# q8888620002/Group-Attribution-for-Diffusion-Models

Measured on AMD Instinct MI355X. Metric: shapley_coalitions_per_hour, higher is better.
Workload: dtype f32; 1 GPU; CIFAR-20 DDPM sFT coalition (BASELINE configs[1]): gd_steps=1000 @B=128 + 10240 samples x 100 DDIM steps @B=32 (32 batches fused/launch), UNet2DModel widths [128, 256, 256, 256] 35.75M params fp32; step = 1/1000 coalition = 1 train step + 1 sampler step @B=1024, enqueued on 3 HIP streams (the train step belongs to a later coalition: independent work); coalitions_in_flight=3

## Files before the change

group-attribution-for-diffusion-models_amd/csrc/norm.hip:

```cpp
#include "gad_common.h"
#include "gad_reduce.h"
#include "gemm_dev.h"

namespace {

constexpr int NT = 256;
constexpr int MAXC = 3072;

struct Geo {
  int B, HW, C, G, cpg, C4, tpr, rows_par, nch, ppc;
};

static Geo make_geo(const gad_groupnorm_args* a) {
  Geo g;
  g.B = a->B; g.HW = a->HW; g.C = a->C; g.G = a->G;
  g.cpg = a->C / a->G;
  g.C4 = a->C / 4;
  g.tpr = g.C4 < NT ? g.C4 : NT;
  g.rows_par = NT / g.tpr;
  int nch = 2048 / (a->B > 0 ? a->B : 1);
  int maxch = a->HW / (8 * g.rows_par > 32 ? 8 * g.rows_par : 32);
  if (nch > maxch) nch = maxch;
  if (nch < 1) nch = 1;
  g.ppc = (a->HW + nch - 1) / nch;
// ... 156 lines not shown
    f32x4 mu, rs;
#pragma unroll
    for (int e = 0; e < 4; ++e) {
      int grp = (c0 + e) / g.cpg;
      mu[e] = s_mean[grp];
      rs[e] = s_rstd[grp];
    }
    f32x4 scale = rs * ga, shift = be - mu * scale;
    const bool far = gn_far_mean(mu, rs);
    long base = ((long)b * g.HW) * g.C + c0;
    int ldx;
    const float* xb = gn_src(x, x2, C1, g.C, g.HW, b, c0, &ldx);
    int p = p0 + prow;
    const int R = g.rows_par;
    for (; p + 3 * R < p1; p += 4 * R) {
      f32x4 v[4];
#pragma unroll
      for (int u = 0; u < 4; ++u) v[u] = *reinterpret_cast<const f32x4*>(xb + (long)(p + u * R) * ldx);
#pragma unroll
      for (int u = 0; u < 4; ++u) {
        f32x4 z = far ? (v[u] - mu) * scale + be : v[u] * scale + shift;
        if (silu) {
#pragma unroll
          for (int e = 0; e < 4; ++e) z[e] = silu_f(z[e]);
        }
        *reinterpret_cast<f32x4*>(y + base + (long)(p + u * R) * g.C) = z;
      }
    }
    for (; p < p1; p += R) {
      f32x4 v = *reinterpret_cast<const f32x4*>(xb + (long)p * ldx);
      f32x4 z = far ? (v - mu) * scale + be : v * scale + shift;
      if (silu) {
#pragma unroll
        for (int e = 0; e < 4; ++e) z[e] = silu_f(z[e]);
      }
      *reinterpret_cast<f32x4*>(y + base + (long)p * g.C) = z;
    }
  }
}


struct SlabGeo {
  int HW, C, G, cpg, SC, qpr, PL, P2, nslab, gps, qpg;
  int xgrp;
};
__device__ __forceinline__ void slab_of_block(const SlabGeo& s, int& b, int& sl) {
  const int bid = blockIdx.x;
  if (s.xgrp) {
    const int x = bid & 7, r = bid >> 3;
    const int bp = r / s.nslab;
    sl = r - bp * s.nslab;
    b = bp * 8 + x;
  } else {
    b = bid / s.nslab;
    sl = bid - b * s.nslab;
  }
}

__device__ __forceinline__ void slab_reduce(float* red, float val, const SlabGeo& s, int pl, bool act) {
  red[threadIdx.x] = val;
  for (int st = s.P2 >> 1; st >= 1; st >>= 1) {
    __syncthreads();
    if (act && pl < st && pl + st < s.PL) red[threadIdx.x] += red[threadIdx.x + st * s.qpr];
  }
  __syncthreads();
}

template <int NTH>
__device__ __forceinline__ void slab_reduce4(f32x4* red, f32x4 val, const SlabGeo& s, int pl, bool act) {
  red[threadIdx.x] = val;
  for (int st = s.P2 >> 1; st >= 1; st >>= 1) {
    __syncthreads();
    if (act && pl < st && pl + st < s.PL) red[threadIdx.x] += red[threadIdx.x + st * s.qpr];
  }
  __syncthreads();
}

template <int NV, bool PERCH = false, int NTH = NT>
__global__ __launch_bounds__(NTH) void gn_slab_kernel(const float* __restrict__ x, const float* __restrict__ x2, int C1,
                                                     float* __restrict__ y,
                                                     const float* __restrict__ gamma, const float* __restrict__ beta,
                                                     float* __restrict__ mean_out, float* __restrict__ rstd_out,
                                                     SlabGeo s, float eps, int silu) {
  __shared__ float red[PERCH ? 4 : NTH];
  __shared__ f32x4 red4[PERCH ? NTH : 1];
  __shared__ float s_mean[64], s_rstd[64];
  int b, sl;
  slab_of_block(s, b, sl);
  const int tid = threadIdx.x;
  const int pl = tid / s.qpr, q = tid - pl * s.qpr;
  const bool act = pl < s.PL;
  const int c0 = sl * s.SC + q * 4;
  const long base = ((long)b * s.HW) * s.C + c0;
  const bool second = c0 >= C1;
  const int ldin = second ? s.C - C1 : C1;
  const float* xin = (second ? x2 + (c0 - C1) : x + c0) + ((long)b * s.HW) * ldin;
  f32x4 v[NV];
#pragma unroll
  for (int i = 0; i < NV; ++i) {
    int p = pl + i * s.PL;
    v[i] = (act && p < s.HW) ? *reinterpret_cast<const f32x4*>(xin + (long)p * ldin) : f32x4{0.f, 0.f, 0.f, 0.f};
  }
  f32x4 acc = {0.f, 0.f, 0.f, 0.f};
#pragma unroll
  for (int i = 0; i < NV; ++i) acc += v[i];
  const float inv_n = 1.f / (float)((long)s.HW * s.cpg);
  const float* chan = reinterpret_cast<const float*>(red4);
  int gi[4] = {0, 0, 0, 0};
  if (PERCH) {
#pragma unroll
    for (int e = 0; e < 4; ++e) gi[e] = act ? (q * 4 + e) / s.cpg : 0;
    slab_reduce4<NTH>(red4, acc, s, pl, act);
  } else {
    slab_reduce(red, (acc[0] + acc[1]) + (acc[2] + acc[3]), s, pl, act);
  }
  float S = 0.f;
  if (tid < s.gps) {
    if (PERCH) for (int j = 0; j < s.cpg; ++j) S += chan[tid * s.cpg + j];
    else for (int j = 0; j < s.qpg; ++j) S += red[tid * s.qpg + j];
    s_mean[tid] = S * inv_n;
  }
  __syncthreads();
  f32x4 mu;
  if (PERCH) mu = f32x4{s_mean[gi[0]], s_mean[gi[1]], s_mean[gi[2]], s_mean[gi[3]]};
  else { const float m1 = act ? s_mean[q / s.qpg] : 0.f; mu = f32x4{m1, m1, m1, m1}; }
  acc = f32x4{0.f, 0.f, 0.f, 0.f};
#pragma unroll
  for (int i = 0; i < NV; ++i) {
    int p = pl + i * s.PL;
    f32x4 d = v[i] - mu;
    if (act && p < s.HW) acc += d * d;
  }
  if (PERCH) {
    __syncthreads();
    slab_reduce4<NTH>(red4, acc, s, pl, act);
  } else {
    slab_reduce(red, (acc[0] + acc[1]) + (acc[2] + acc[3]), s, pl, act);
  }
  if (tid < s.gps) {
    float SS = 0.f;
    if (PERCH) for (int j = 0; j < s.cpg; ++j) SS += chan[tid * s.cpg + j];
    else for (int j = 0; j < s.qpg; ++j) SS += red[tid * s.qpg + j];
    float rs = rsqrtf(SS * inv_n + eps);
    if (!((s_mean[tid] * rs) * (s_mean[tid] * rs) <= GN_COND - 1.f)) {
      const float md = S / (float)((long)s.HW * s.cpg), d = s_mean[tid] - md;
      rs = rsqrtf(fmaxf(SS * inv_n - d * d, 0.f) + eps);
      s_mean[tid] = md;
    }
    s_rstd[tid] = rs;
    mean_out[b * s.G + sl * s.gps + tid] = s_mean[tid];
    rstd_out[b * s.G + sl * s.gps + tid] = rs;
  }
  __syncthreads();
  if (!act) return;
  f32x4 rs;
  if (PERCH) {
    rs = f32x4{s_rstd[gi[0]], s_rstd[gi[1]], s_rstd[gi[2]], s_rstd[gi[3]]};
    mu = f32x4{s_mean[gi[0]], s_mean[gi[1]], s_mean[gi[2]], s_mean[gi[3]]};
  } else {
    const float r1 = s_rstd[q / s.qpg], m1 = s_mean[q / s.qpg];
    rs = f32x4{r1, r1, r1, r1};
    mu = f32x4{m1, m1, m1, m1};
  }
  f32x4 ga = *reinterpret_cast<const f32x4*>(gamma + c0), be = *reinterpret_cast<const f32x4*>(beta + c0);
  f32x4 scale = ga * rs, shift = be - scale * mu;
  const bool far = gn_far_mean(mu, rs);
#pragma unroll
  for (int i = 0; i < NV; ++i) {
    int p = pl + i * s.PL;
    if (p < s.HW) {
      f32x4 z = far ? (v[i] - mu) * scale + be : v[i] * scale + shift;
      if (silu) {
#pragma unroll
        for (int e = 0; e < 4; ++e) z[e] = silu_f(z[e]);
      }
      *reinterpret_cast<f32x4*>(y + base + (long)p * s.C) = z;
    }
  }
}

static int make_slab(const gad_groupnorm_args* a, SlabGeo* out, const int nth = NT, const int maxnv = 32) {
  const int cpg = a->C / a->G;
  SlabGeo best{};
  int best_nv = 0;
  long best_score = -1;
  for (int k = 1; k * cpg <= a->C && k <= 64; ++k) {
    int SC = k * cpg;
    if (a->C % SC != 0 || SC % 4 != 0) continue;
    const bool lines = (SC * 4) % 128 == 0 || SC == a->C;
    if (!lines && (a->B % 8 != 0 || a->C / SC > 8 || (long)a->B * (a->C / SC) > 1024)) continue;
    int qpr = SC / 4;
    if (qpr > nth) break;
    int PL = nth / qpr;
    int nv = (a->HW + PL - 1) / PL;
    if (nv > maxnv) continue;
    long blocks = (long)a->B * (a->C / SC);
    long score = (blocks >= 1024 ? (1L << 40) : blocks << 16) + SC + (lines ? (1L << 41) : 0);
    if (score > best_score) {
      best_score = score;
      best_nv = nv;
      int P2 = 1;
      while (P2 < PL) P2 <<= 1;
      best = SlabGeo{a->HW, a->C, a->G, cpg, SC, qpr, PL, P2, a->C / SC, k, cpg / 4, lines ? 0 : 1};
    }
  }
  if (!best_nv) return 0;
  *out = best;
  return best_nv <= 4 ? 4 : best_nv <= 8 ? 8 : best_nv <= 16 ? 16 : 32;
}

struct GnWino {
  float* V;
  int W, TH, TW;
  long pos_stride;
};

template <int NV>
__global__ __launch_bounds__(512) void gn_wino4_kernel(const float* __restrict__ x, const float* __restrict__ x2, int C1,
                                                      const float* __restrict__ gamma, const float* __restrict__ beta,
                                                      float* __restrict__ mean_out, float* __restrict__ rstd_out,
                                                      SlabGeo s, float eps, int silu, GnWino w) {
  constexpr int NTH = 512;
  extern __shared__ __attribute__((aligned(16))) float gn_img[];
  __shared__ float red[NTH];
  __shared__ float s_mean[64], s_rstd[64];
  int b, sl;
  slab_of_block(s, b, sl);
  const int tid = threadIdx.x;
  const int pl = tid / s.qpr, q = tid - pl * s.qpr;
  const bool act = pl < s.PL;
  const int c0 = sl * s.SC + q * 4;
  const bool second = c0 >= C1;
  const int ldin = second ? s.C - C1 : C1;
  const float* xin = (second ? x2 + (c0 - C1) : x + c0) + ((long)b * s.HW) * ldin;
  f32x4 v[NV];
#pragma unroll
  for (int i = 0; i < NV; ++i) {
    int p = pl + i * s.PL;
    v[i] = (act && p < s.HW) ? *reinterpret_cast<const f32x4*>(xin + (long)p * ldin) : f32x4{0.f, 0.f, 0.f, 0.f};
  }
  f32x4 acc = {0.f, 0.f, 0.f, 0.f};
#pragma unroll
  for (int i = 0; i < NV; ++i) acc += v[i];
  const float inv_n = 1.f / (float)((long)s.HW * s.cpg);
  slab_reduce(red, (acc[0] + acc[1]) + (acc[2] + acc[3]), s, pl, act);
  float S = 0.f;
  if (tid < s.gps) {
    for (int j = 0; j < s.qpg; ++j) S += red[tid * s.qpg + j];
    s_mean[tid] = S * inv_n;
  }
  __syncthreads();
  const float m1 = act ? s_mean[q / s.qpg] : 0.f;
  const f32x4 mu = f32x4{m1, m1, m1, m1};
  acc = f32x4{0.f, 0.f, 0.f, 0.f};
#pragma unroll
  for (int i = 0; i < NV; ++i) {
    int p = pl + i * s.PL;
    f32x4 d = v[i] - mu;
    if (act && p < s.HW) acc += d * d;
  }
  slab_reduce(red, (acc[0] + acc[1]) + (acc[2] + acc[3]), s, pl, act);
  if (tid < s.gps) {
    float SS = 0.f;
    for (int j = 0; j < s.qpg; ++j) SS += red[tid * s.qpg + j];
    float rs = rsqrtf(SS * inv_n + eps);
    if (!((s_mean[tid] * rs) * (s_mean[tid] * rs) <= GN_COND - 1.f)) {
      const float md = S / (float)((long)s.HW * s.cpg), d = s_mean[tid] - md;
      rs = rsqrtf(fmaxf(SS * inv_n - d * d, 0.f) + eps);
      s_mean[tid] = md;
    }
    s_rstd[tid] = rs;
    mean_out[b * s.G + sl * s.gps + tid] = s_mean[tid];
    rstd_out[b * s.G + sl * s.gps + tid] = rs;
  }
  __syncthreads();
  f32x4* img4 = reinterpret_cast<f32x4*>(gn_img);
  if (act) {
    const float r1 = s_rstd[q / s.qpg], m2 = s_mean[q / s.qpg];
    const f32x4 rs = f32x4{r1, r1, r1, r1}, mu2 = f32x4{m2, m2, m2, m2};
    const f32x4 ga = *reinterpret_cast<const f32x4*>(gamma + c0), be = *reinterpret_cast<const f32x4*>(beta + c0);
    const f32x4 scale = ga * rs, shift = be - scale * mu2;
    const bool far = gn_far_mean(mu2, rs);
#pragma unroll
    for (int i = 0; i < NV; ++i) {
      int p = pl + i * s.PL;
      if (p < s.HW) {
        f32x4 z = far ? (v[i] - mu2) * scale + be : v[i] * scale + shift;
        if (silu) {
#pragma unroll
          for (int e = 0; e < 4; ++e) z[e] = silu_f(z[e]);
        }
        const int yy = p / w.W, xx = p - yy * w.W;
        img4[(yy * w.W + (xx ^ ((xx >> 2) & 1))) * s.qpr + q] = z;
      }
    }
  }
  __syncthreads();
  const int H = s.HW / w.W;
  const int items = w.TH * w.TW * s.qpr;
  for (int it = tid; it < items; it += NTH) {
    const int tile = it / s.qpr, qq = it - tile * s.qpr;
    const int ty = tile / w.TW, tx = tile - ty * w.TW;
    f32x4 t[6][6];
#pragma unroll
    for (int dx = 0; dx < 6; ++dx) {
      const int xx = 4 * tx - 1 + dx;
      const bool xok = xx >= 0 && xx < w.W;
      const int xs = xx ^ ((xx >> 2) & 1);
      f32x4 d[6], col[6];
#pragma unroll
      for (int dy = 0; dy < 6; ++dy) {
        const int yy = 4 * ty - 1 + dy;
        const bool ok = xok && yy >= 0 && yy < H;
        d[dy] = ok ? img4[(yy * w.W + xs) * s.qpr + qq] : f32x4{0.f, 0.f, 0.f, 0.f};
      }
      gadk::wino4_bt(d, col);
#pragma unroll
      for (int i = 0; i < 6; ++i) t[i][dx] = col[i];
    }
    float* out = w.V + ((long)b * (w.TH * w.TW) + tile) * s.C + sl * s.SC + qq * 4;
#pragma unroll
    for (int i = 0; i < 6; ++i) {
      f32x4 vv[6];
      gadk::wino4_bt(t[i], vv);
#pragma unroll
      for (int j = 0; j < 6; ++j) *reinterpret_cast<f32x4*>(out + (long)(6 * i + j) * w.pos_stride) = vv[j];
    }
  }
}

static int make_slab_wino(const gad_groupnorm_args* a, SlabGeo* out) {
  const int cpg = a->C / a->G, nth = 512;
  if (cpg % 4 != 0) return 0;
  int best_nv = 0;
  long best_score = -1;
  for (int k = 1; k * cpg <= a->C && k <= 64; ++k) {
    const int SC = k * cpg;
    if (a->C % SC != 0 || SC % 32 != 0) continue;
    if ((long)a->HW * SC * 4 > 128 * 1024) break;
    const int qpr = SC / 4;
    if (qpr > nth) break;
    const int PL = nth / qpr, nv = (a->HW + PL - 1) / PL;
    if (nv > 16) continue;
    const long blocks = (long)a->B * (a->C / SC);
    const long score = (blocks >= 512 ? (1L << 40) : blocks << 16) + SC;
    if (score > best_score) {
      best_score = score;
      best_nv = nv;
      int P2 = 1;
      while (P2 < PL) P2 <<= 1;
      *out = SlabGeo{a->HW, a->C, a->G, cpg, SC, qpr, PL, P2, a->C / SC, k, cpg / 4, 0};
    }
  }
  return !best_nv ? 0 : best_nv <= 4 ? 4 : best_nv <= 8 ? 8 : 16;
}

__device__ __forceinline__ float act_grad(float dy, float z, int silu) {
  if (!silu) return dy;
  float s = 1.f / (1.f + expf(-z));
  return dy * s * (1.f + z * (1.f - s));
}

template <int NV, int NTH>
__global__ __launch_bounds__(NTH) void gn_bwd_slab_kernel(const float* __restrict__ x, const float* __restrict__ dy,
                                                          float* __restrict__ dx, const float* __restrict__ gamma,
                                                          const float* __restrict__ beta, const float* __restrict__ mean,
                                                          const float* __restrict__ rstd, float* __restrict__ part,
                                                          SlabGeo s, int silu, const float* __restrict__ dx_add) {
  __shared__ f32x4 red_a[NTH], red_b[NTH];
  __shared__ float s_m1[64], s_m2[64];
  int b, sl;
  slab_of_block(s, b, sl);
  const int tid = threadIdx.x;
  const int pl = tid / s.qpr, q = tid - pl * s.qpr;
  const bool act = pl < s.PL;
  const int c0 = sl * s.SC + (act ? q : 0) * 4;
  const long base = ((long)b * s.HW) * s.C + c0;
  int gi[4];
  f32x4 mu, rs;
#pragma unroll
  for (int e = 0; e < 4; ++e) {
    gi[e] = ((act ? q : 0) * 4 + e) / s.cpg;
    mu[e] = mean[b * s.G + sl * s.gps + gi[e]];
    rs[e] = rstd[b * s.G + sl * s.gps + gi[e]];
  }
  const f32x4 ga = *reinterpret_cast<const f32x4*>(gamma + c0), be = *reinterpret_cast<const f32x4*>(beta + c0);
  f32x4 xh[NV], ge[NV];
  f32x4 sa = {0.f, 0.f, 0.f, 0.f}, sb = {0.f, 0.f, 0.f, 0.f};
#pragma unroll
  for (int i = 0; i < NV; ++i) {
    const int p = pl + i * s.PL;
    if (act && p < s.HW) {
      const f32x4 v = *reinterpret_cast<const f32x4*>(x + base + (long)p * s.C);
      const f32x4 d = *reinterpret_cast<const f32x4*>(dy + base + (long)p * s.C);
      xh[i] = (v - mu) * rs;
#pragma unroll
      for (int e = 0; e < 4; ++e) ge[i][e] = act_grad(d[e], xh[i][e] * ga[e] + be[e], silu);
      sa += ge[i];
      sb += ge[i] * xh[i];
    } else {
      xh[i] = f32x4{0.f, 0.f, 0.f, 0.f};
      ge[i] = f32x4{0.f, 0.f, 0.f, 0.f};
    }
  }
  slab_reduce4<NTH>(red_a, sa, s, pl, act);
  slab_reduce4<NTH>(red_b, sb, s, pl, act);
  if (tid < s.qpr) {
    const int c = sl * s.SC + tid * 4;
    float* o = part + ((long)b * s.C + c) * 2;
    const f32x4 A = red_a[tid], Bx = red_b[tid];
#pragma unroll
    for (int e = 0; e < 4; ++e) { o[2 * e] = A[e]; o[2 * e + 1] = Bx[e]; }
  }
  if (tid < s.gps) {
    const float inv_n = 1.f / (float)((long)s.HW * s.cpg);
    const float* ca = reinterpret_cast<const float*>(red_a);
    const float* cb = reinterpret_cast<const float*>(red_b);
    float s1 = 0.f, s2 = 0.f;
    for (int j = 0; j < s.cpg; ++j) {
      const int c = tid * s.cpg + j;
      const float gj = gamma[sl * s.SC + c];
      s1 += ca[c] * gj;
      s2 += cb[c] * gj;
    }
    s_m1[tid] = s1 * inv_n;
    s_m2[tid] = s2 * inv_n;
  }
  __syncthreads();
  if (!act) return;
  const f32x4 m1 = {s_m1[gi[0]], s_m1[gi[1]], s_m1[gi[2]], s_m1[gi[3]]}, m2 = {s_m2[gi[0]], s_m2[gi[1]], s_m2[gi[2]], s_m2[gi[3]]};
#pragma unroll
  for (int i = 0; i < NV; ++i) {
    const int p = pl + i * s.PL;
    if (p < s.HW) {
      f32x4 o;
#pragma unroll
      for (int e = 0; e < 4; ++e) o[e] = rs[e] * (ge[i][e] * ga[e] - m1[e] - xh[i][e] * m2[e]);
      if (dx_add) o += *reinterpret_cast<const f32x4*>(dx_add + base + (long)p * s.C);
      *reinterpret_cast<f32x4*>(dx + base + (long)p * s.C) = o;
    }
  }
}

__global__ __launch_bounds__(NT) void gn_bwd_stats_kernel(const float* __restrict__ x, const float* __restrict__ dy,
                                                          const float* __restrict__ gamma, const float* __restrict__ beta,
                                                          const float* __restrict__ mean, const float* __restrict__ rstd,
                                                          float* __restrict__ part, Geo g, int silu) {
  __shared__ float red[2 * MAXC];
  int b = blockIdx.x / g.nch, ch = blockIdx.x - b * g.nch;
  int p0 = ch * g.ppc, p1 = min(g.HW, p0 + g.ppc);
  int tid = threadIdx.x;
  int prow = tid / g.tpr, cfirst = tid - prow * g.tpr;
  if (prow < g.rows_par) {
    for (int cq = cfirst; cq < g.C4; cq += g.tpr) {
      int c0 = cq * 4;
      f32x4 ga = *reinterpret_cast<const f32x4*>(gamma + c0), be = *reinterpret_cast<const f32x4*>(beta + c0);
      f32x4 mu, rs;
#pragma unroll
      for (int e = 0; e < 4; ++e) {
        int grp = (c0 + e) / g.cpg;
        mu[e] = mean[b * g.G + grp];
        rs[e] = rstd[b * g.G + grp];
      }
      f32x4 sa = {0, 0, 0, 0}, sb = {0, 0, 0, 0};
      long base = ((long)b * g.HW) * g.C + c0;
      for (int p = p0 + prow; p < p1; p += g.rows_par) {
        f32x4 v = *reinterpret_cast<const f32x4*>(x + base + (long)p * g.C);
        f32x4 d = *reinterpret_cast<const f32x4*>(dy + base + (long)p * g.C);
        f32x4 xh = (v - mu) * rs;
#pragma unroll
        for (int e = 0; e < 4; ++e) {
          float ge = act_grad(d[e], xh[e] * ga[e] + be[e], silu);
          sa[e] += ge;
          sb[e] += ge * xh[e];
        }
      }
      float* r0 = red + prow * g.C + c0;
      float* r1 = red + g.rows_par * g.C + prow * g.C + c0;
#pragma unroll
      for (int e = 0; e < 4; ++e) { r0[e] = sa[e]; r1[e] = sb[e]; }
    }
  }
  __syncthreads();
  for (int c = tid; c < g.C; c += NT) {
    float A = 0.f, Bx = 0.f;
    for (int r = 0; r < g.rows_par; ++r) {
      A += red[r * g.C + c];
      Bx += red[g.rows_par * g.C + r * g.C + c];
    }
    float* o = part + (((long)b * g.nch + ch) * g.C + c) * 2;
    o[0] = A;
    o[1] = Bx;
  }
}

__global__ __launch_bounds__(NT) void gn_bwd_apply_kernel(const float* __restrict__ x, const float* __restrict__ dy,
                                                          float* __restrict__ dx, const float* __restrict__ gamma,
                                                          const float* __restrict__ beta, const float* __restrict__ mean,
                                                          const float* __restrict__ rstd, const float* __restrict__ part,
                                                          Geo g, int silu, const float* __restrict__ dx_add) {
  __shared__ float s_a[MAXC], s_b[MAXC];
  __shared__ float s_s1[256], s_s2[256];
  int b = blockIdx.x / g.nch, ch = blockIdx.x - b * g.nch;
  int tid = threadIdx.x;
  for (int c = tid; c < g.C; c += NT) {
    float A = 0.f, Bx = 0.f;
    for (int k = 0; k < g.nch; ++k) {
      const float* o = part + (((long)b * g.nch + k) * g.C + c) * 2;
      A += o[0];
      Bx += o[1];
    }
    float ga = gamma[c];
    s_a[c] = A * ga;
    s_b[c] = Bx * ga;
  }
  __syncthreads();
  for (int grp = tid; grp < g.G; grp += NT) {
    float s1 = 0.f, s2 = 0.f;
    for (int c = grp * g.cpg; c < (grp + 1) * g.cpg; ++c) {
      s1 += s_a[c];
      s2 += s_b[c];
    }
    float inv_n = 1.f / (float)((long)g.HW * g.cpg);
    s_s1[grp] = s1 * inv_n;
    s_s2[grp] = s2 * inv_n;
  }
  __syncthreads();
  int prow = tid / g.tpr, cfirst = tid - prow * g.tpr;
  if (prow >= g.rows_par) return;
  int p0 = ch * g.ppc, p1 = min(g.HW, p0 + g.ppc);
  for (int cq = cfirst; cq < g.C4; cq += g.tpr) {
    int c0 = cq * 4;
    f32x4 ga = *reinterpret_cast<const f32x4*>(gamma + c0), be = *reinterpret_cast<const f32x4*>(beta + c0);
    f32x4 mu, rs, m1, m2;
#pragma unroll
    for (int e = 0; e < 4; ++e) {
      int grp = (c0 + e) / g.cpg;
      mu[e] = mean[b * g.G + grp];
      rs[e] = rstd[b * g.G + grp];
      m1[e] = s_s1[grp];
      m2[e] = s_s2[grp];
    }
    long base = ((long)b * g.HW) * g.C + c0;
    for (int p = p0 + prow; p < p1; p += g.rows_par) {
      f32x4 v = *reinterpret_cast<const f32x4*>(x + base + (long)p * g.C);
      f32x4 d = *reinterpret_cast<const f32x4*>(dy + base + (long)p * g.C);
      f32x4 xh = (v - mu) * rs, o;
#pragma unroll
      for (int e = 0; e < 4; ++e) {
        float ge = act_grad(d[e], xh[e] * ga[e] + be[e], silu);
        o[e] = rs[e] * (ge * ga[e] - m1[e] - xh[e] * m2[e]);
      }
      if (dx_add) o += *reinterpret_cast<const f32x4*>(dx_add + base + (long)p * g.C);
      *reinterpret_cast<f32x4*>(dx + base + (long)p * g.C) = o;
    }
  }
}

static int check(const gad_groupnorm_args* a, const char* who) {
  GAD_CHECK(a && a->x && a->y && a->gamma && a->beta && a->mean && a->rstd, "%s: null pointer", who);
  GAD_CHECK(a->B > 0 && a->HW > 0 && a->C > 0 && a->G > 0 && a->C % a->G == 0, "%s: bad shape", who);
  GAD_CHECK(a->C % 4 == 0 && a->C <= MAXC && a->G <= 256, "%s: needs C%%4==0, C<=3072, G<=256 (C=%d G=%d)", who, a->C, a->G);
  GAD_CHECK(gad_aligned16(a->x) && gad_aligned16(a->y) && gad_aligned16(a->gamma) && gad_aligned16(a->beta), "%s: pointers must be 16-byte aligned", who);
  int64_t need = gad_groupnorm_workspace_bytes(a);
  GAD_CHECK(a->ws && a->ws_bytes >= need, "%s: workspace too small (%lld < %lld)", who, (long long)a->ws_bytes, (long long)need);
  return 0;
}

}

extern "C" int64_t gad_groupnorm_workspace_bytes(const gad_groupnorm_args* a) {
  Geo g = make_geo(a);
  int64_t parts = (int64_t)a->B * g.nch * a->C * 2 * (int64_t)sizeof(float);
  const int64_t r1 = gad_reduce::ws_bytes(1, (long)a->B * g.nch, 2 * a->C);
  const int64_t r2 = gad_reduce::ws_bytes(1, (long)a->B, 2 * a->C);
  return parts + (r1 > r2 ? r1 : r2);
}

extern "C" int gad_groupnorm_one_pass(const gad_groupnorm_args* a) {
  if (!a || a->B <= 0 || a->HW <= 0 || a->C <= 0 || a->G <= 0 || a->C % a->G != 0 || a->C % 4 != 0) return 0;
  if (a->flags & GAD_GN_TWO_PASS) return 0;
  SlabGeo sg;
  return make_slab(a, &sg) ? 1 : 0;
}

extern "C" int gad_groupnorm_silu_fwd(const gad_groupnorm_args* a, void* stream) {
  if (check(a, "gad_groupnorm_silu_fwd")) return 1;
  hipStream_t st = (hipStream_t)stream;
  SlabGeo sg;
  int nv = (a->flags & GAD_GN_TWO_PASS) ? 0 : make_slab(a, &sg);
  if (a->x2)
    GAD_CHECK(a->C1 > 0 && a->C1 < a->C && a->C1 % 4 == 0 && (a->C - a->C1) % 4 == 0 && gad_aligned16(a->x2), "gad_groupnorm_silu_fwd: bad C1 / x2");
  if (nv) {
    const int c1 = a->x2 ? a->C1 : a->C;
    dim3 sgrid(a->B * sg.nslab), sblock(NT);
    const bool perch = (a->C / a->G) % 4 != 0;
    SlabGeo sgw;
    if (nv == 32 && !perch && make_slab(a, &sgw, 512, 16) == 16 && sgw.SC == sg.SC) {
      dim3 wgrid(a->B * sgw.nslab);
      hipLaunchKernelGGL((gn_slab_kernel<16, false, 512>), wgrid, dim3(512), 0, st, a->x, a->x2, c1, a->y, a->gamma, a->beta,
                         a->mean, a->rstd, sgw, a->eps, a->silu);
      GAD_LAUNCH_CHECK("gn_slab(512)");
      return 0;
    }
#define GAD_GNF(NV_, P_) hipLaunchKernelGGL((gn_slab_kernel<NV_, P_>), sgrid, sblock, 0, st, a->x, a->x2, c1, a->y, a->gamma, a->beta, \
                                            a->mean, a->rstd, sg, a->eps, a->silu)
    switch (nv) {
      case 4: if (perch) GAD_GNF(4, true); else GAD_GNF(4, false); break;
      case 8: if (perch) GAD_GNF(8, true); else GAD_GNF(8, false); break;
      case 16: if (perch) GAD_GNF(16, true); else GAD_GNF(16, false); break;
      default: if (perch) GAD_GNF(32, true); else GAD_GNF(32, false); break;
    }
#undef GAD_GNF
    GAD_LAUNCH_CHECK("gn_slab");
    return 0;
  }
  Geo g = make_geo(a);
  dim3 grid(a->B * g.nch), block(NT);
  hipLaunchKernelGGL(gn_stats_kernel, grid, block, 0, st, a->x, (float*)a->ws, g, a->x2, a->C1);
  GAD_LAUNCH_CHECK("gn_stats");
  hipLaunchKernelGGL(gn_apply_kernel, grid, block, 0, st, a->x, a->y, a->gamma, a->beta, (const float*)a->ws, a->mean, a->rstd, g, a->eps, a->silu,
                     a->x2, a->C1);
  GAD_LAUNCH_CHECK("gn_apply");
  return 0;
}


static bool gn_wino_shapes_ok(const gad_groupnorm_args* a, int32_t W) {
  if (!a || a->B <= 0 || a->HW <= 0 || a->C <= 0 || a->G <= 0 || a->C % a->G != 0 || a->C % 32 != 0 || a->G > 256) return false;
  if (W <= 0 || a->HW % W != 0 || (W & 3) || ((a->HW / W) & 3)) return false;
  if (a->x2 && !(a->C1 > 0 && a->C1 < a->C && a->C1 % 4 == 0 && (a->C - a->C1) % 4 == 0)) return false;
  return true;
}
extern "C" int gad_groupnorm_wino4_ok(const gad_groupnorm_args* a, int32_t W) {
  SlabGeo sg;
  return gn_wino_shapes_ok(a, W) && make_slab_wino(a, &sg) ? 1 : 0;
}
extern "C" int gad_groupnorm_silu_wino4(const gad_groupnorm_args* a, float* V, int32_t W, void* stream) {
  GAD_CHECK(a && a->x && a->gamma && a->beta && a->mean && a->rstd && V, "gad_groupnorm_silu_wino4: null pointer");
  GAD_CHECK(gn_wino_shapes_ok(a, W), "gad_groupnorm_silu_wino4: shapes outside the plan (C %% 32, W and H multiples of 4; C=%d G=%d HW=%d W=%d)", a->C, a->G, a->HW, W);
  GAD_CHECK(gad_aligned16(a->x) && gad_aligned16(V) && gad_aligned16(a->gamma) && gad_aligned16(a->beta) && (!a->x2 || gad_aligned16(a->x2)),
            "gad_groupnorm_silu_wino4: pointers must be 16-byte aligned");
  SlabGeo sg;
  const int nv = make_slab_wino(a, &sg);
  GAD_CHECK(nv, "gad_groupnorm_silu_wino4: no slab plan (gad_groupnorm_wino4_ok tells)");
  GnWino w;
  w.V = V; w.W = W; w.TH = (a->HW / W) / 4; w.TW = W / 4;
  w.pos_stride = (long)a->B * w.TH * w.TW * a->C;
  const int c1 = a->x2 ? a->C1 : a->C;
  const int bytes = a->HW * sg.SC * (int)sizeof(float);
  hipStream_t st = (hipStream_t)stream;
  dim3 grid(a->B * sg.nslab), block(512);
#define GAD_GNW(NV_)                                                                                                        \
  do {                                                                                                                      \
    static int lds_set = 0;                                                                                                 \
    if (bytes > lds_set) {                                                                                                  \
      hipError_t e = hipFuncSetAttribute(reinterpret_cast<const void*>(gn_wino4_kernel<NV_>), hipFuncAttributeMaxDynamicSharedMemorySize, bytes); \
      GAD_CHECK(e == hipSuccess, "gad_groupnorm_silu_wino4: cannot reserve %d bytes of LDS: %s", bytes, hipGetErrorString(e)); \
      lds_set = bytes;                                                                                                      \
    }                                                                                                                       \
    hipLaunchKernelGGL((gn_wino4_kernel<NV_>), grid, block, bytes, st, a->x, a->x2, c1, a->gamma, a->beta, a->mean, a->rstd, sg, a->eps, a->silu, w); \
  } while (0)
  if (nv == 4) GAD_GNW(4);
  else if (nv == 8) GAD_GNW(8);
  else GAD_GNW(16);
#undef GAD_GNW
  GAD_LAUNCH_CHECK("gn_wino4");
  return 0;
}

extern "C" int gad_groupnorm_silu_bwd(const gad_groupnorm_args* a, void* stream) {
  if (check(a, "gad_groupnorm_silu_bwd")) return 1;
  GAD_CHECK(a->dy && gad_aligned16(a->dy) && ((a->dgamma == nullptr) == (a->dbeta == nullptr)), "gad_groupnorm_silu_bwd: null/unaligned grad pointer");
  GAD_CHECK(!a->dx_add || gad_aligned16(a->dx_add), "gad_groupnorm_silu_bwd: dx_add must be 16-byte aligned");
  Geo g = make_geo(a);
  hipStream_t st = (hipStream_t)stream;
  if (!(a->flags & GAD_GN_TWO_PASS)) {
    SlabGeo sg;
    int nth = NT, nv = make_slab(a, &sg, NT, 16);
    if (!nv) { nth = 512; nv = make_slab(a, &sg, 512, 16); }
    if (nv) {
      float* part = (float*)a->ws;
      dim3 sgrid(a->B * sg.nslab);
#define GAD_GNB(NV_, NTH_) hipLaunchKernelGGL((gn_bwd_slab_kernel<NV_, NTH_>), sgrid, dim3(NTH_), 0, st, a->x, a->dy, a->y, a->gamma, \
                                              a->beta, a->mean, a->rstd, part, sg, a->silu, a->dx_add)
      if (nth == NT) {
        if (nv <= 4) GAD_GNB(4, NT);
        else GAD_GNB(16, NT);
      } else {
        GAD_GNB(16, 512);
      }
#undef GAD_GNB
      GAD_LAUNCH_CHECK("gn_bwd_slab");
      if (a->dgamma) {
        float* ws2 = part + (long)a->B * a->C * 2;
        gad_reduce::launch(part, a->dbeta, a->dgamma, 1, (long)a->B, 2 * a->C, ws2, st);
        GAD_LAUNCH_CHECK("gn_bwd_param");
      }
      return 0;
    }
  }
  dim3 grid(a->B * g.nch), block(NT);
  hipLaunchKernelGGL(gn_bwd_stats_kernel, grid, block, 0, st, a->x, a->dy, a->gamma, a->beta, a->mean, a->rstd, (float*)a->ws, g, a->silu);
  GAD_LAUNCH_CHECK("gn_bwd_stats");
  hipLaunchKernelGGL(gn_bwd_apply_kernel, grid, block, 0, st, a->x, a->dy, a->y, a->gamma, a->beta, a->mean, a->rstd, (const float*)a->ws, g, a->silu, a->dx_add);
  GAD_LAUNCH_CHECK("gn_bwd_apply");
  if (a->dgamma) {
    float* ws2 = (float*)a->ws + (long)a->B * g.nch * a->C * 2;
    gad_reduce::launch((const float*)a->ws, a->dbeta, a->dgamma, 1, (long)a->B * g.nch, 2 * a->C, ws2, st);
    GAD_LAUNCH_CHECK("gn_bwd_param");
  }
  return 0;
}
```

group-attribution-for-diffusion-models_amd/gad/ops.py:

```python
from __future__ import annotations

import ctypes as C
import math
from typing import Optional

import torch

from . import _capi
from ._capi import (A_CONV, A_CONVT, A_KC, A_MC, B_CONV, B_KC, B_MC, B_WDGRAD, AdamArgs, ConvGeom, GemmArgs,
                    GroupNormArgs, check)

_WS = {}
WS_BYTES = 1 << 30


def _stream():
    return C.c_void_p(torch.cuda.current_stream().cuda_stream)


_raw_stream = getattr(torch._C, "_cuda_getCurrentRawStream", None)


WS_OVERRIDE = [None]

# ... 231 lines not shown
        check(lib.gad_gemm_plan(C.byref(a), C.byref(tile), C.byref(sk), C.byref(vec)), "gad_gemm_plan")
        kid = lib.gad_gemm_kernel_id(C.byref(a))
        s, e, mid = torch.cuda.Event(enable_timing=True), torch.cuda.Event(enable_timing=True), None
        s.record()
        if kid in (5, 6) and not (a.flags & _capi.GEMM_WINO_SKIP_INPUT):
            flags = a.flags
            mid = torch.cuda.Event(enable_timing=True)
            a.flags = flags | _capi.GEMM_WINO_ONLY_INPUT
            check(lib.gad_gemm(C.byref(a), _stream()), "gad_gemm")
            mid.record()
            a.flags = flags | _capi.GEMM_WINO_SKIP_INPUT
            check(lib.gad_gemm(C.byref(a), _stream()), "gad_gemm")
            a.flags = flags
        else:
            check(lib.gad_gemm(C.byref(a), _stream()), "gad_gemm")
        e.record()
        name = self.NAMES.get((a.a_mode, a.b_mode), "gemm") + ("", "_bf16", f"_patch_w{a.g.Wo}", f"_patch_bf16_w{a.g.Wo}", f"_fewout_valu_w{a.g.Wo}", "_wino", "_wino4", "_wino4")[kid]
        key = (name, tile.value, sk.value, vec.value)
        g = a.g
        if a.a_mode in (A_CONV, A_CONVT):
            a_elems = (a.M // max(1, g.Ho * g.Wo)) * g.H * g.W * g.C
        else:
            a_elems = a.M * a.K
        b_elems = (a.K // max(1, g.Ho * g.Wo)) * g.H * g.W * g.C if a.b_mode == B_CONV else a.N * a.K
        extra = a.M * a.N if a.residual else 0
        nbytes = 4.0 * max(1, batch) * (a_elems + b_elems + a.M * a.N + extra)
        flops = 2.0 * a.M * a.N * a.K * max(1, batch)
        executed = flops * ({5: 16.0 / 36.0, 6: 0.25, 7: 0.25}.get(kid, 1.0))
        stage = None
        if kid in (5, 6):
            npos, tpx = (16, 4) if kid == 5 else (36, 16)
            v_bytes = 4.0 * npos * (a.M // tpx) * g.C
            stage = (mid, 4.0 * a_elems + v_bytes if mid is not None else 0.0, v_bytes + 4.0 * (b_elems * npos / 9.0 + a.M * a.N + extra))
        self.records.append((key, flops, nbytes, s, e, executed, stage))

    def hgemm(self, lib, a, tn=False):
        s, e = torch.cuda.Event(enable_timing=True), torch.cuda.Event(enable_timing=True)
        if tn:
            s.record()
            check(lib.gad_hgemm_tn(C.byref(a), _stream()), "gad_hgemm_tn")
            e.record()
            nbytes = 2.0 * a.K * (a.M + a.N) + 4.0 * a.M * a.N
            flops = 2.0 * a.M * a.N * a.K
            self.records.append((("hgemm_tn_wgrad", 128, 0, 8), flops, nbytes, s, e, flops, None))
            return
        tile, sk = C.c_int32(), C.c_int32()
        check(lib.gad_hgemm_plan(C.byref(a), C.byref(tile), C.byref(sk)), "gad_hgemm_plan")
        s.record()
        check(lib.gad_hgemm(C.byref(a), _stream()), "gad_hgemm")
        e.record()
        if a.conv:
            name = f"hconv{a.KH}x{a.KW}" + ("_s2dgrad" if a.conv == 2 else "_s2" if a.stride == 2 else "_up" if a.upsample else "")
            a_elems = (a.M // max(1, a.Ho * a.Wo)) * a.H * a.W * a.Cin
        else:
            name = "hgemm_wgrad" if a.out_f32 else "hgemm_lora" if a.A2 else "hgemm"
            a_elems = a.M * a.K
        nbytes = 2.0 * (a_elems + a.N * a.K + (a.M * a.N if a.residual else 0)) + (4.0 if a.out_f32 else 2.0) * a.M * a.N
        flops = 2.0 * a.M * a.N * a.K
        self.records.append(((name, {1: 128, 2: 320, 5: 256320, 6: 256320, 7: 320, 8: 128, 9: 128}[tile.value], sk.value, 8), flops, nbytes, s, e, flops, None))

    def attention(self, fn, a, what, elem_bytes=4):
        s, e = torch.cuda.Event(enable_timing=True), torch.cuda.Event(enable_timing=True)
        s.record()
        check(fn(C.byref(a), _stream()), f"gad_attention_{what}")
        e.record()
        d_alg = getattr(a, "alg_d", a.d)
        unit = float(a.B) * a.heads * a.Tq * a.Tk * d_alg
        qb, kb = float(elem_bytes) * a.B * a.Tq * a.heads * d_alg, float(elem_bytes) * a.B * a.Tk * a.heads * d_alg
        flops, nbytes = (4.0 * unit, 2 * qb + 2 * kb) if what == "fwd" else (10.0 * unit, 4 * qb + 4 * kb)
        self.records.append(((f"attn_{what}_d{d_alg}", a.Tq, a.Tk, elem_bytes), flops, nbytes, s, e, flops, None))

    def summary(self):
        out = {}
        for key, fl, nb, s, e, ex, stage in self.records:
            d = out.setdefault(key, dict(launches=0, ms=0.0, flops=0.0, bytes=0.0, executed=0.0))
            d["launches"] += 1
            d["ms"] += s.elapsed_time(e)
            d["flops"] += fl
            d["bytes"] += nb
            d["executed"] += ex
            if stage is not None:
                d["bytes_rest"] = d.get("bytes_rest", 0.0) + stage[2]
                d.setdefault("ms_input", 0.0)
                d.setdefault("bytes_input", 0.0)
                d.setdefault("n_input", 0)
                if stage[0] is not None:
                    d["ms_input"] += s.elapsed_time(stage[0])
                    d["bytes_input"] += stage[1]
                    d["n_input"] += 1
        return out


PROFILER = None


def _conv_out_size(h, k, stride, pad_lo, pad_hi):
    return (h + pad_lo + pad_hi - k) // stride + 1


def conv2d_fwd_raw(x, w, bias, stride=1, pad=(1, 1, 1, 1), upsample=False, rowadd=None, residual=None,
                   tile_hint=0, splitk_hint=0, x2=None, wino_input=None, keep_v=None):
    _req(x, "conv x")
    Bn, H, W, C1 = x.shape
    Cin = C1
    if x2 is not None:
        _req(x2, "conv x2")
        if x2.shape[:3] != x.shape[:3]:
            raise _capi.GadError(f"conv x2 {tuple(x2.shape)} does not match x {tuple(x.shape)}")
        Cin = C1 + x2.shape[-1]
    wk = weight_krsc(w)
    Cout, KH, KW, wc = wk.shape
    if wc != Cin:
        raise _capi.GadError(f"conv weight expects {wc} input channels, got {Cin}")
    He, We = (2 * H, 2 * W) if upsample else (H, W)
    Ho = _conv_out_size(He, KH, stride, pad[0], pad[1])
    Wo = _conv_out_size(We, KW, stride, pad[2], pad[3])
    y = _out((Bn, Ho, Wo, Cout), x.device)
    g = ConvGeom(H, W, Cin, C1, Ho, Wo, KH, KW, stride, pad[0], pad[2], int(upsample))
    if residual is not None:
        _req(residual, "conv residual")
    wino_ok = (KH == 3 and KW == 3 and stride == 1 and x2 is None and tile_hint in (0, 7, 8, 9, 10, 11) and splitk_hint == 0
               and tuple(pad) == (1, 1, 1, 1))
    f4_maps = Ho % 4 == 0 and Wo % 4 == 0 and not KERNEL_FLAGS.get("no_wino4")
    launched = gemm_raw(x, wk, y, A_CONV, B_KC, Bn * Ho * Wo, Cout, KH * KW * Cin, 0, KH * KW * Cin, Cout, geom=g,
             bias=bias, rowadd=rowadd, rows_per_group=Ho * Wo, residual=residual, ldr=Cout,
             tile_hint=tile_hint, splitk_hint=splitk_hint, A2=x2, a_split=C1, wino_input=wino_input, keep_v=keep_v,
             B_wino=wino_weight(w, 2) if (wino_ok and (tile_hint == 7 or (tile_hint == 0 and not f4_maps))) else None,
             B_wino4=wino_weight(w, 4) if (wino_ok and tile_hint != 7 and f4_maps) else None,
             B_bf16=bf16_weight(w) if (OPERAND_PRECISION[0] >= 1 and KH == 3 and Cin % 32 == 0 and x2 is None
                                       and not torch.cuda.is_current_stream_capturing()) else None)
    return y if launched is not False else None


def gn_silu_conv3x3_raw(x, x2, gamma, beta, G, eps, w, bias, rowadd=None, residual=None, tile_hint=0):
    _req(x, "groupnorm x")
    Bn, H, W, C1 = x.shape
    Cin = C1 + (x2.shape[-1] if x2 is not None else 0)
    lib = _capi.load()

    def plain():
        h = group_norm_cat_raw(x, x2, gamma, beta, G, eps, True) if x2 is not None else group_norm(x, gamma, beta, G, eps, True)
        return conv2d_fwd_raw(h, w, bias, 1, (1, 1, 1, 1), False, rowadd=rowadd, residual=residual, tile_hint=tile_hint)
    if (torch.is_grad_enabled() or tuple(w.shape[2:]) != (3, 3) or w.shape[1] != Cin or OPERAND_PRECISION[0] != 0 or KERNEL_FLAGS["gn"]
            or KERNEL_FLAGS.get("no_gn_wino") or H % 4 or W % 4):
        return plain()
    mean = torch.empty((Bn, G), device=x.device, dtype=torch.float32)
    rstd = torch.empty_like(mean)
    a = GroupNormArgs()
    a.x, a.gamma, a.beta, a.mean, a.rstd = x.data_ptr(), gamma.data_ptr(), beta.data_ptr(), mean.data_ptr(), rstd.data_ptr()
    a.B, a.HW, a.C, a.G, a.eps, a.silu = Bn, H * W, Cin, G, eps, 1
    if x2 is not None:
        _req(x2, "groupnorm x2")
        a.x2, a.C1 = x2.data_ptr(), C1
    if not lib.gad_groupnorm_wino4_ok(C.byref(a), W):
        return plain()

    def fill(V):
        check(lib.gad_groupnorm_silu_wino4(C.byref(a), V.data_ptr(), W, _stream()), "gad_groupnorm_silu_wino4")
    y = conv2d_fwd_raw(_ShapeOnly(x, (Bn, H, W, Cin)), w, bias, 1, (1, 1, 1, 1), False, rowadd=rowadd, residual=residual,
                       tile_hint=tile_hint, wino_input=fill)
    return y if y is not None else plain()


class _ShapeOnly:

    def __init__(self, t, shape):
        self._t, self.shape, self.device, self.dtype = t, tuple(shape), t.device, t.dtype
        self.is_cuda = t.is_cuda

    def data_ptr(self):
        return self._t.data_ptr()

    def is_contiguous(self):
        return True


def bf16_weight(w):
    home = getattr(w, "_gad_flat", None)
    if home is not None and w.data_ptr() == home[0].data_ptr() + 4 * home[1]:
        flat, off, n = home
        key = (flat._version, WEIGHT_EPOCH[0], getattr(flat, "_gad_epoch", 0))
        cached = getattr(flat, "_gad_bf16", None)
        if cached is None or cached[0] != key:
            shadow = cached[1] if cached is not None else torch.empty(flat.numel(), device=flat.device, dtype=torch.bfloat16)
            shadow.copy_(flat.detach())
            cached = (key, shadow, {o_: p_._version for p_, o_, _ in getattr(flat, "_gad_params", ())})
            flat._gad_bf16 = cached
        if cached[2].get(off, w._version) != w._version:
            cached[1][off:off + n].copy_(flat.detach()[off:off + n])
            cached[2][off] = w._version
        o, i, kh, kw = w.shape
        return cached[1][off:off + n].view(o, kh, kw, i)
    key = weight_key(w)
    cached = getattr(w, "_gad_bf16", None)
    if cached is None or cached[0] != key:
        cached = (key, weight_krsc(w).detach().to(torch.bfloat16).contiguous())
        w._gad_bf16 = cached
    return cached[1]


def _in_flat_buffer(w) -> bool:
    home = getattr(w, "_gad_flat", None)
    return home is not None and w.data_ptr() == home[0].data_ptr() + 4 * home[1]


def dgrad_as_forward(w, stride, pad) -> bool:
    return (tuple(w.shape[2:]) == (3, 3) and stride == 1 and tuple(pad) == (1, 1, 1, 1) and w.shape[0] % 32 == 0
            and w.shape[1] >= 64 and (not w.requires_grad or _in_flat_buffer(w)) and not KERNEL_FLAGS.get("native_dgrad"))


def _rot_table(flat):
    cached = getattr(flat, "_gad_rot_table", None)
    if cached is None:
        rows = [(off, p_.shape[0], p_.shape[1], a, b)
                for p_, off, _ in getattr(flat, "_gad_params", ()) if p_.ndim == 4 and tuple(p_.shape[2:]) == (3, 3)
                for a in range(0, p_.shape[0], 32) for b in range(0, p_.shape[1], 32)]
        cached = (torch.tensor(rows, dtype=torch.int64, device=flat.device), len(rows)) if rows else (None, 0)
        flat._gad_rot_table = cached
    return cached


def rotated_weight(w):
    if _in_flat_buffer(w):
        flat, off, n = w._gad_flat
        table, tiles = _rot_table(flat)
        key = (flat._version, WEIGHT_EPOCH[0], getattr(flat, "_gad_epoch", 0))
        cached = getattr(flat, "_gad_rot", None)
        stale = cached is None or cached[0] != key
        if not stale and cached[2].get(off, w._version) != w._version:
            stale = True
        if stale and tiles:
            shadow = cached[1] if cached is not None else torch.empty_like(flat)
            shadow._gad_conv3x3 = [(o_, b, a) for o_, a, b in _conv3x3_residents(flat)]
            check(_capi.load().gad_rotate_conv3x3(flat.data_ptr(), shadow.data_ptr(), table.data_ptr(), tiles, _stream()),
                  "gad_rotate_conv3x3")
            shadow._gad_epoch = getattr(shadow, "_gad_epoch", 0) + 1
            cached = (key, shadow, {o_: p_._version for p_, o_, _ in flat._gad_params}, cached[3] if cached is not None else {})
            flat._gad_rot = cached
        view = cached[3].get(off)
        if view is None:
            co, ci = w.shape[0], w.shape[1]
            view = cached[1][off:off + n].view(ci, 3, 3, co).permute(0, 3, 1, 2)
            view._gad_flat = (cached[1], off, n)
            cached[3][off] = view
        return view
    key = weight_key(w)
    cached = getattr(w, "_gad_rot", None)
    if cached is None or cached[0] != key:
        store = weight_krsc(w).detach().flip(1, 2).permute(3, 1, 2, 0).contiguous()
        cached = (key, store.permute(0, 3, 1, 2))
        w._gad_rot = cached
    return cached[1]


def _conv3x3_residents(flat):
    r = getattr(flat, "_gad_conv3x3", None)
    if r is None:
        r = [(off, p_.shape[0], p_.shape[1]) for p_, off, _ in getattr(flat, "_gad_params", ())
             if p_.ndim == 4 and tuple(p_.shape[2:]) == (3, 3)]
        flat._gad_conv3x3 = r
    return r


def _wino_ok(co, ci):
    return ci % 32 == 0 and co % 4 == 0 and co >= 64


def _wino_transform(src, items, npos):
    rows, where, doff = [], {}, 0
    for off, co, ci in items:
        where[off] = (doff, npos * co * ci)
        rows += [(off, doff, co, ci, a, b) for a in range(0, co, 32) for b in range(0, ci, 32)]
        doff += npos * co * ci
    U = torch.empty(max(doff, 1), device=src.device, dtype=torch.float32)
    table = torch.tensor(rows, dtype=torch.int64, device=src.device)
    return U, where, table, len(rows)


def wino_weight(w, f=2):
    co, ci = w.shape[0], w.shape[1]
    if (tuple(w.shape[2:]) != (3, 3) or not _wino_ok(co, ci) or OPERAND_PRECISION[0] >= 1
            or KERNEL_FLAGS["gemm"] & (_capi.GEMM_NO_WINO | _capi.GEMM_NO_PATCH | _capi.GEMM_SCALAR_EPILOGUE | _capi.GEMM_TAP_MAJOR_K)
            or (f == 4 and KERNEL_FLAGS.get("no_wino4"))):
        return None
    lib = _capi.load()
    launch, npos, attr = (lib.gad_wino_weights, 16, "_gad_wino") if f == 2 else (lib.gad_wino4_weights, 36, "_gad_wino4")
    if _in_flat_buffer(w):
        flat, off, n = w._gad_flat
        key = (flat._version, WEIGHT_EPOCH[0], getattr(flat, "_gad_epoch", 0))
        cached = getattr(flat, attr, None)
        if cached is None:
            items = [(o_, a, b) for o_, a, b in _conv3x3_residents(flat) if _wino_ok(a, b)]
            cached = [None, *_wino_transform(flat, items, npos), {}]
            setattr(flat, attr, cached)
        _, U, where, table, tiles, versions = cached
        if off not in where:
            return None
        stale = cached[0] != key or versions.get(off, w._version) != w._version
        if stale:
            check(launch(flat.data_ptr(), U.data_ptr(), table.data_ptr(), tiles, _stream()), "gad_wino_weights")
            cached[0] = key
            cached[5] = {o_: p_._version for p_, o_, _ in getattr(flat, "_gad_params", ())}
        d0, dn = where[off]
        return U[d0:d0 + dn]
    key = weight_key(w)
    cached = getattr(w, attr, None)
# ... 970 lines not shown
```

Before: 45.45 coalitions/hour.

## Add streaming GroupNorm+SiLU Winograd input-transform path when no slab plan fits

Adds a fallback for the fused GroupNorm/SiLU/Winograd-input-transform path when the LDS slab plan cannot hold the tensor. It runs the stats pass only (writing no normalized output), then a new kernel that combines the partials, normalizes, applies SiLU and writes the Winograd B^T d B tiles straight to V. This skips materializing the normalized activation and a separate transform pass for large-HW layers. The cost is rereading overlapping 6x6 input tiles and recombining partials in every block.

After: 45.46 coalitions/hour, median of 2. Within noise of the previous version (+0.0%).

```diff
diff --git a/group-attribution-for-diffusion-models_amd/csrc/norm.hip b/group-attribution-for-diffusion-models_amd/csrc/norm.hip
--- a/group-attribution-for-diffusion-models_amd/csrc/norm.hip
+++ b/group-attribution-for-diffusion-models_amd/csrc/norm.hip
@@ -332,7 +332,7 @@
     rstd_out[b * s.G + sl * s.gps + tid] = rs;
   }
   __syncthreads();
-  if (!act) return;
+  if (!act || y == nullptr) return;
   f32x4 rs;
   if (PERCH) {
     rs = f32x4{s_rstd[gi[0]], s_rstd[gi[1]], s_rstd[gi[2]], s_rstd[gi[3]]};
@@ -535,6 +535,82 @@
   return !best_nv ? 0 : best_nv <= 4 ? 4 : best_nv <= 8 ? 8 : 16;
 }
 
+__global__ __launch_bounds__(NT) void gn_wino4_stream_kernel(const float* __restrict__ x, const float* __restrict__ x2, int C1,
+                                                             const float* __restrict__ gamma, const float* __restrict__ beta,
+                                                             const float* __restrict__ part, float* mean_out, float* rstd_out,
+                                                             Geo g, float eps, int silu, GnWino w, int bpi) {
+  __shared__ float s_mean[256], s_rstd[256];
+  const int b = blockIdx.x / bpi, blk = blockIdx.x - b * bpi;
+  const int tid = threadIdx.x;
+  if (part) {
+    gn_combine(part, g, b, eps, s_mean, s_rstd);
+    __syncthreads();
+    if (blk == 0)
+      for (int grp = tid; grp < g.G; grp += NT) {
+        mean_out[b * g.G + grp] = s_mean[grp];
+        rstd_out[b * g.G + grp] = s_rstd[grp];
+      }
+  } else {
+    for (int grp = tid; grp < g.G; grp += NT) {
+      s_mean[grp] = mean_out[b * g.G + grp];
+      s_rstd[grp] = rstd_out[b * g.G + grp];
+    }
+    __syncthreads();
+  }
+  const int per = w.TH * w.TW;
+  const int it = blk * NT + tid;
+  if (it >= per * g.C4) return;
+  const int tile = it / g.C4, c0 = (it - tile * g.C4) * 4;
+  const int ty = tile / w.TW, tx = tile - ty * w.TW;
+  const int H = g.HW / w.W;
+  const f32x4 ga = *reinterpret_cast<const f32x4*>(gamma + c0), be = *reinterpret_cast<const f32x4*>(beta + c0);
+  f32x4 mu, rs;
+#pragma unroll
+  for (int e = 0; e < 4; ++e) {
+    const int grp = (c0 + e) / g.cpg;
+    mu[e] = s_mean[grp];
+    rs[e] = s_rstd[grp];
+  }
+  const f32x4 scale = rs * ga, shift = be - mu * scale;
+  const bool far = gn_far_mean(mu, rs);
+  int ldx;
+  const float* xb = gn_src(x, x2, C1, g.C, g.HW, b, c0, &ldx);
+  f32x4 t[6][6];
+#pragma unroll
+  for (int dx = 0; dx < 6; ++dx) {
+    const int xx = 4 * tx - 1 + dx;
+    const bool xok = xx >= 0 && xx < w.W;
+    f32x4 d[6], col[6];
+    bool ok[6];
+#pragma unroll
+    for (int dy = 0; dy < 6; ++dy) {
+      const int yy = 4 * ty - 1 + dy;
+      ok[dy] = xok && yy >= 0 && yy < H;
+      d[dy] = ok[dy] ? *reinterpret_cast<const f32x4*>(xb + ((long)yy * w.W + xx) * ldx) : f32x4{0.f, 0.f, 0.f, 0.f};
+    }
+#pragma unroll
+    for (int dy = 0; dy < 6; ++dy) {
+      f32x4 z = far ? (d[dy] - mu) * scale + be : d[dy] * scale + shift;
+      if (silu) {
+#pragma unroll
+        for (int e = 0; e < 4; ++e) z[e] = silu_f(z[e]);
+      }
+      d[dy] = ok[dy] ? z : f32x4{0.f, 0.f, 0.f, 0.f};
+    }
+    gadk::wino4_bt(d, col);
+#pragma unroll
+    for (int i = 0; i < 6; ++i) t[i][dx] = col[i];
+  }
+  float* out = w.V + ((long)b * per + tile) * g.C + c0;
+#pragma unroll
+  for (int i = 0; i < 6; ++i) {
+    f32x4 vv[6];
+    gadk::wino4_bt(t[i], vv);
+#pragma unroll
+    for (int j = 0; j < 6; ++j) *reinterpret_cast<f32x4*>(out + (long)(6 * i + j) * w.pos_stride) = vv[j];
+  }
+}
+
 __device__ __forceinline__ float act_grad(float dy, float z, int silu) {
   if (!silu) return dy;
   float s = 1.f / (1.f + expf(-z));
@@ -764,13 +840,10 @@
   return make_slab(a, &sg) ? 1 : 0;
 }
 
-extern "C" int gad_groupnorm_silu_fwd(const gad_groupnorm_args* a, void* stream) {
-  if (check(a, "gad_groupnorm_silu_fwd")) return 1;
-  hipStream_t st = (hipStream_t)stream;
+static int gn_fwd_launch(const gad_groupnorm_args* a, float* y, hipStream_t st, bool* partials) {
   SlabGeo sg;
   int nv = (a->flags & GAD_GN_TWO_PASS) ? 0 : make_slab(a, &sg);
-  if (a->x2)
-    GAD_CHECK(a->C1 > 0 && a->C1 < a->C && a->C1 % 4 == 0 && (a->C - a->C1) % 4 == 0 && gad_aligned16(a->x2), "gad_groupnorm_silu_fwd: bad C1 / x2");
+  if (partials) *partials = !nv;
   if (nv) {
     const int c1 = a->x2 ? a->C1 : a->C;
     dim3 sgrid(a->B * sg.nslab), sblock(NT);
@@ -778,12 +851,12 @@
     SlabGeo sgw;
     if (nv == 32 && !perch && make_slab(a, &sgw, 512, 16) == 16 && sgw.SC == sg.SC) {
       dim3 wgrid(a->B * sgw.nslab);
-      hipLaunchKernelGGL((gn_slab_kernel<16, false, 512>), wgrid, dim3(512), 0, st, a->x, a->x2, c1, a->y, a->gamma, a->beta,
+      hipLaunchKernelGGL((gn_slab_kernel<16, false, 512>), wgrid, dim3(512), 0, st, a->x, a->x2, c1, y, a->gamma, a->beta,
                          a->mean, a->rstd, sgw, a->eps, a->silu);
       GAD_LAUNCH_CHECK("gn_slab(512)");
       return 0;
     }
-#define GAD_GNF(NV_, P_) hipLaunchKernelGGL((gn_slab_kernel<NV_, P_>), sgrid, sblock, 0, st, a->x, a->x2, c1, a->y, a->gamma, a->beta, \
+#define GAD_GNF(NV_, P_) hipLaunchKernelGGL((gn_slab_kernel<NV_, P_>), sgrid, sblock, 0, st, a->x, a->x2, c1, y, a->gamma, a->beta, \
                                             a->mean, a->rstd, sg, a->eps, a->silu)
     switch (nv) {
       case 4: if (perch) GAD_GNF(4, true); else GAD_GNF(4, false); break;
@@ -799,10 +872,18 @@
   dim3 grid(a->B * g.nch), block(NT);
   hipLaunchKernelGGL(gn_stats_kernel, grid, block, 0, st, a->x, (float*)a->ws, g, a->x2, a->C1);
   GAD_LAUNCH_CHECK("gn_stats");
-  hipLaunchKernelGGL(gn_apply_kernel, grid, block, 0, st, a->x, a->y, a->gamma, a->beta, (const float*)a->ws, a->mean, a->rstd, g, a->eps, a->silu,
+  if (!y) return 0;
+  hipLaunchKernelGGL(gn_apply_kernel, grid, block, 0, st, a->x, y, a->gamma, a->beta, (const float*)a->ws, a->mean, a->rstd, g, a->eps, a->silu,
                      a->x2, a->C1);
   GAD_LAUNCH_CHECK("gn_apply");
   return 0;
+}
+
+extern "C" int gad_groupnorm_silu_fwd(const gad_groupnorm_args* a, void* stream) {
+  if (check(a, "gad_groupnorm_silu_fwd")) return 1;
+  if (a->x2)
+    GAD_CHECK(a->C1 > 0 && a->C1 < a->C && a->C1 % 4 == 0 && (a->C - a->C1) % 4 == 0 && gad_aligned16(a->x2), "gad_groupnorm_silu_fwd: bad C1 / x2");
+  return gn_fwd_launch(a, a->y, (hipStream_t)stream, nullptr);
 }
 
 
@@ -812,9 +893,13 @@
   if (a->x2 && !(a->C1 > 0 && a->C1 < a->C && a->C1 % 4 == 0 && (a->C - a->C1) % 4 == 0)) return false;
   return true;
 }
+static bool gn_stream_ok(const gad_groupnorm_args* a) {
+  if (a->C > MAXC || !a->ws || a->ws_bytes < gad_groupnorm_workspace_bytes(a)) return false;
+  return (int64_t)a->B * gad_ceil_div((int64_t)(a->HW / 16) * (a->C / 4), NT) < (1L << 31);
+}
 extern "C" int gad_groupnorm_wino4_ok(const gad_groupnorm_args* a, int32_t W) {
   SlabGeo sg;
-  return gn_wino_shapes_ok(a, W) && make_slab_wino(a, &sg) ? 1 : 0;
+  return gn_wino_shapes_ok(a, W) && (make_slab_wino(a, &sg) || gn_stream_ok(a)) ? 1 : 0;
 }
 extern "C" int gad_groupnorm_silu_wino4(const gad_groupnorm_args* a, float* V, int32_t W, void* stream) {
   GAD_CHECK(a && a->x && a->gamma && a->beta && a->mean && a->rstd && V, "gad_groupnorm_silu_wino4: null pointer");
@@ -823,11 +908,22 @@
             "gad_groupnorm_silu_wino4: pointers must be 16-byte aligned");
   SlabGeo sg;
   const int nv = make_slab_wino(a, &sg);
-  GAD_CHECK(nv, "gad_groupnorm_silu_wino4: no slab plan (gad_groupnorm_wino4_ok tells)");
+  GAD_CHECK(nv || gn_stream_ok(a), "gad_groupnorm_silu_wino4: no slab plan, and no workspace for the streaming plan (gad_groupnorm_wino4_ok tells)");
   GnWino w;
   w.V = V; w.W = W; w.TH = (a->HW / W) / 4; w.TW = W / 4;
   w.pos_stride = (long)a->B * w.TH * w.TW * a->C;
   const int c1 = a->x2 ? a->C1 : a->C;
+  if (!nv) {
+    hipStream_t st = (hipStream_t)stream;
+    bool partials = false;
+    if (int rc = gn_fwd_launch(a, nullptr, st, &partials)) return rc;
+    const Geo g = make_geo(a);
+    const int bpi = (int)gad_ceil_div((int64_t)w.TH * w.TW * g.C4, NT);
+    hipLaunchKernelGGL(gn_wino4_stream_kernel, dim3((unsigned)(a->B * bpi)), dim3(NT), 0, st, a->x, a->x2, c1, a->gamma, a->beta,
+                       partials ? (const float*)a->ws : nullptr, a->mean, a->rstd, g, a->eps, a->silu, w, bpi);
+    GAD_LAUNCH_CHECK("gn_wino4_stream");
+    return 0;
+  }
   const int bytes = a->HW * sg.SC * (int)sizeof(float);
   hipStream_t st = (hipStream_t)stream;
   dim3 grid(a->B * sg.nslab), block(512);
diff --git a/group-attribution-for-diffusion-models_amd/gad/ops.py b/group-attribution-for-diffusion-models_amd/gad/ops.py
--- a/group-attribution-for-diffusion-models_amd/gad/ops.py
+++ b/group-attribution-for-diffusion-models_amd/gad/ops.py
@@ -407,6 +407,8 @@
     if x2 is not None:
         _req(x2, "groupnorm x2")
         a.x2, a.C1 = x2.data_ptr(), C1
+    ws = workspace(x.device) if SCRATCH_ALLOC is None else _scratch("ws", lib.gad_groupnorm_workspace_bytes(C.byref(a)), x.device)
+    a.ws, a.ws_bytes = ws.data_ptr(), ws.numel()
     if not lib.gad_groupnorm_wino4_ok(C.byref(a), W):
         return plain()
 
```
